# NVIDIA/k8s-cc-manager

Hardware: AMD Instinct MI355X
Metric: reconcile_gpus_per_sec (higher is better)
Workload: dtype bf16; 1 GPU; model=cc-mode-transition, global_batch=1, seq_len=1024, parallelism=concurrent-per-gpu x1, modes=on<->off toggle, device_tier=shadow+hip-attest, eviction=True, components=5, attest_gemm_dim=1024

## Files before the change

k8s_cc_manager_amd/ops/attest.py:

```python

from __future__ import annotations

import ctypes
import logging
import os
import re
from dataclasses import dataclass, fields
from pathlib import Path
from typing import Optional

logger = logging.getLogger(__name__)

_LIB_PATH = Path(__file__).resolve().parent / "libccattest.so"
_lib: Optional[ctypes.CDLL] = None


class AttestationError(Exception):
    """The post-reset attestation probe failed — the device must NOT be
    labeled ready."""


def _from_c(cls, c, **special):
    special.update(error=c.error.decode(errors="replace"), ok=bool(c.ok))
    return cls(**{f.name: special[f.name] if f.name in special
# ... 188 lines not shown
        ("bad_offset", ctypes.c_ulonglong * 16),
        ("bad_expected", ctypes.c_uint * 16),
        ("bad_got", ctypes.c_uint * 16),
        ("bad_pass", ctypes.c_int * 16),
        ("fill_ms", ctypes.c_double),
        ("flip_ms", ctypes.c_double),
        ("scrub_ms", ctypes.c_double),
        ("zero_ms", ctypes.c_double),
        ("alloc_ms", ctypes.c_double),
        ("gbps", ctypes.c_double),
        ("beyond_cache", ctypes.c_int),
        ("scrubbed", ctypes.c_int),
        ("ok", ctypes.c_int),
        ("error", ctypes.c_char * 256),
    ]


HBM_MUL_LO, HBM_MUL_HI, HBM_SALT = 2654435769, 2246822519, 0x5EED0001
_HBM_NO_OFFSET = (1 << 64) - 1


def hbm_pattern_word(w: int, phase: int) -> int:
    if phase == 2:
        return 0
    if phase not in (0, 1):
        raise ValueError(f"phase={phase} outside 0..2")
    p = ((w & 0xFFFFFFFF) * HBM_MUL_LO + (w >> 32) * HBM_MUL_HI
         + HBM_SALT) & 0xFFFFFFFF
    return p ^ 0xFFFFFFFF if phase else p


@dataclass
class HbmMarchReport:

    device: int
    bytes_requested: int
    bytes_tested: int
    chunk_bytes: int
    origin: int
    chunks: int
    passes: int
    mismatch_words: int
    first_bad_offset: Optional[int]
    bad: list
    fill_ms: float
    flip_ms: float
    scrub_ms: float
    zero_ms: float
    alloc_ms: float
    gbps: float
    beyond_cache: bool
    scrubbed: bool
    ok: bool
    error: str = ""

    @classmethod
    def from_c(cls, c: _CHbmReport) -> "HbmMarchReport":
        n = max(0, min(c.n_bad, len(c.bad_offset)))
        first = c.first_bad_offset
        return _from_c(
            cls, c,
            first_bad_offset=None if first == _HBM_NO_OFFSET else first,
            bad=[(c.bad_offset[i], c.bad_expected[i], c.bad_got[i],
                  c.bad_pass[i]) for i in range(n)],
            beyond_cache=bool(c.beyond_cache), scrubbed=bool(c.scrubbed))


_INT, _PTR = ctypes.c_int, ctypes.c_void_p
_I64, _U64 = ctypes.c_longlong, ctypes.c_ulonglong
_GEMM =[_INT, _PTR, _PTR, _PTR, _INT, _INT, _INT]
_MX_GEMM = [_INT] + [_PTR] * 5 + [_INT] * 3
_UNIT_TABLE = [_INT, ctypes.POINTER(ctypes.c_uint), _INT]

_BINDINGS = {
    "cc_device_alive": (_INT, [_INT]),
    "cc_device_count": (_INT, []),
    "cc_device_index_for_bdf": (_INT, [_INT] * 3),
    "cc_mfma_gemm_bf16": (_INT, _GEMM),
    "cc_mfma_gemm_bf16_variant": (_INT, _GEMM + [_INT]),
    "cc_mfma_gemm_fp8_variant": (_INT, _GEMM + [_INT]),
    "cc_mfma_gemm_fp8": (_INT, _GEMM),
    "cc_ref_gemm_f32": (_INT, _GEMM),
    "cc_attest_device": (_INT, [_INT, _INT, ctypes.POINTER(_CReport)]),
    "cc_report_sizeof": (_INT, []),
    "cc_mfma_gemm_mxfp4": (_INT, _MX_GEMM),
    "cc_ref_gemm_mxfp4_f32": (_INT, _MX_GEMM),
    "cc_attest_mxfp4": (_INT, [_INT, _INT, ctypes.POINTER(_CMxReport)]),
    "cc_mx_report_sizeof": (_INT, []),
    "cc_cu_sweep": (_INT, [_INT, _INT, _INT, ctypes.POINTER(_CSweepReport)]),
    "cc_cu_sweep_gold": (_INT, [_INT, _INT, ctypes.POINTER(ctypes.c_float)]),
    "cc_cu_sweep_units": (_INT, _UNIT_TABLE),
    "cc_cu_sweep_hits": (_INT, _UNIT_TABLE),
    "cc_sweep_report_sizeof": (_INT, []),
    "cc_hbm_march": (_INT, [_INT, _I64, _INT, _U64, _I64, _INT,
                            ctypes.POINTER(_CHbmReport)]),
    "cc_hbm_step": (_INT, [_INT, _PTR, _I64, _U64, _INT, _INT,
                           ctypes.POINTER(_CHbmReport)]),
    "cc_hbm_report_sizeof": (_INT, []),
    "cc_attest_shutdown": (None, []),
}


def _load() -> ctypes.CDLL:
    global _lib
    if _lib is not None:
        return _lib
    if not _LIB_PATH.exists():
        raise AttestationError(
            f"attestation library missing: {_LIB_PATH} — run "
            "python -m k8s_cc_manager_amd.ops.build"
        )
    lib = ctypes.CDLL(str(_LIB_PATH))
    for name, (restype, argtypes) in _BINDINGS.items():
        fn = getattr(lib, name)
        fn.restype, fn.argtypes = restype, argtypes
    _lib = lib
    return lib


def probe_available() -> bool:
    try:
        return _load().cc_device_count() > 0
    except Exception:
        return False


def device_count() -> int:
    return _load().cc_device_count()


def device_alive(device_index: int) -> int:
    return _load().cc_device_alive(device_index)


def shutdown() -> None:
    _load().cc_attest_shutdown()


def attest_device(device_index: int, gemm_dim: int = 1024) -> AttestReport:
    lib = _load()
    c = _CReport()
    rc = lib.cc_attest_device(device_index, gemm_dim, ctypes.byref(c))
    rep = AttestReport.from_c(c)
    if rc != 0:
        raise AttestationError(
            f"device {device_index}: probe runtime error rc={rc}: {rep.error}"
        )
    if not rep.ok:
        raise AttestationError(
            f"device {device_index}: attestation FAILED "
            f"(max_abs_err={rep.max_abs_err}, fp8_max_abs_err={rep.fp8_max_abs_err}, "
            f"lds_failures={rep.lds_failures}, "
            f"xgmi {rep.peers_verified}/{rep.peers_attempted} attempted links verified)"
        )
    logger.info(
        "attested device %d: %s %d CUs, bf16 GEMM %.1f TF/s, fp8 GEMM "
        "%.1f TF/s (%dx%dx%d), LDS ok, HBM %.0f GB/s, xGMI %d/%d peers "
        "(%d verified, %.0f-%.0f GB/s/link)",
        rep.device,
        rep.arch,
        rep.cu_count,
        rep.gemm_tflops,
        rep.fp8_tflops,
        rep.gemm_dim,
        rep.gemm_dim,
        rep.gemm_dim,
        rep.hbm_gbps,
        rep.peers_accessible,
        rep.peer_count,
        rep.peers_verified,
        rep.xgmi_gbps_min,
        rep.xgmi_gbps_max,
    )
    _append_attest_log(rep)
    return rep


def attest_mxfp4(device_index: int, gemm_dim: int = 1024) -> MxReport:
    lib = _load()
    c = _CMxReport()
    rc = lib.cc_attest_mxfp4(device_index, gemm_dim, ctypes.byref(c))
    rep = MxReport.from_c(c)
    if rc != 0:
        raise AttestationError(
            f"device {device_index}: mxfp4 probe runtime error rc={rc}: {rep.error}"
        )
    if not rep.ok:
        raise AttestationError(
            f"device {device_index}: mxfp4 attestation FAILED "
            f"(mx_max_abs_err={rep.mx_max_abs_err}, mx_tflops={rep.mx_tflops})"
        )
    logger.info(
        "attested device %d: mxfp4 GEMM %.1f TF/s (%dx%dx%d), bitwise ok",
        rep.device,
        rep.mx_tflops,
        rep.mx_dim,
        rep.mx_dim,
        rep.mx_dim,
    )
    return rep


CU_SWEEP_MAX_ROUNDS = 256


def unit_name(unit: tuple) -> str:
    return "xcc%d/se%d/sh%d/cu%d/simd%d" % unit


def cu_sweep_report(device_index: int, rounds: int = 32,
                    _poison_key: int = -1) -> CuSweepReport:
    lib = _load()
    c = _CSweepReport()
    rc = lib.cc_cu_sweep(device_index, rounds, _poison_key, ctypes.byref(c))
    rep = CuSweepReport.from_c(c)
    if rc != 0:
        raise AttestationError(
            f"device {device_index}: cu sweep runtime error: {rep.error} rc={rc}"
        )
    return rep


def sweep_compute_units(device_index: int, rounds: int = 32,
                        _poison_key: int = -1) -> CuSweepReport:
    rep = cu_sweep_report(device_index, rounds, _poison_key)
    if not rep.ok:
        if rep.units_failed or rep.lds_failures:
            units = ", ".join(unit_name(u) for u in rep.failed_units)
            more = rep.units_failed - len(rep.failed_units)
            raise AttestationError(
                f"device {device_index}: cu sweep FAILED on {rep.units_failed} "
                f"unit(s): {units}{f' and {more} more' if more > 0 else ''} "
                f"(mfma_failures={rep.mfma_failures}, "
                f"lds_failures={rep.lds_failures})"
            )
        raise AttestationError(
            f"device {device_index}: cu sweep FAILED: {rep.error} "
            f"({rep.cus_seen}/{rep.cu_count} CUs)"
        )
    logger.info(
        "attested device %d: cu sweep %d/%d units on %d CUs of %d XCCs, "
        "%d launch(es), %.2f ms",
        rep.device,
        rep.units_seen,
        rep.units_expected,
        rep.cus_seen,
        rep.xccs_seen,
        rep.launches,
        rep.sweep_ms,
    )
    return rep


def cu_sweep_gold(device_index: int, rounds: int) -> list:
    buf = (ctypes.c_float * SWEEP_GOLD_ELEMS)()
    rc = _load().cc_cu_sweep_gold(device_index, rounds, buf)
    if rc != 0:
        raise AttestationError(f"cu_sweep_gold rc={rc}")
# ... 260 lines not shown
```

k8s_cc_manager_amd/ops/attest_kernels.hip:

```cpp

#include <hip/hip_runtime.h>

#include <chrono>
#include <cstdint>
#include <cstdio>
#include <cstdlib>
#include <mutex>
#include <new>
#include <vector>

#include "gemm_common.hip"
#include "gemm_bf16.hip"
#include "gemm_fp8.hip"
#include "gemm_fp4.hip"
#include "probe_kernels.hip"
#include "cu_sweep.hip"
#include "hbm_march.hip"

#include "probe_reports.hip"
#include "gemm_dispatch.hip"
#include "probe_ctx.hip"
#include "probe_legs.hip"

template <typename Report, typename Refuse = int (*)()>
// ... 18 lines not shown
           origin);
  return -2;
}

extern "C" {

int cc_device_alive(int device) {
  if (device < 0 || device >= kMaxDevices) return -1;
  if (hipSetDevice(device) != hipSuccess) return -1;
  int* d = nullptr;
  {
    std::lock_guard<std::mutex> lk(g_ctx_mu);
    DeviceCtx& dev = device_ctx(device);
    if (dev.dLive.ensure(sizeof(int)) != hipSuccess) return -2;
    d = dev.dLive;
  }
  if (hipMemset(d, 0, sizeof(int)) != hipSuccess) return -2;
  hipLaunchKernelGGL(liveness_kernel, dim3(1), dim3(64), 0, 0, d);
  int h = 0;
  hipError_t e = hipMemcpy(&h, d, sizeof(int), hipMemcpyDeviceToHost);
  if (e != hipSuccess) return -3;
  return h == 0x600D ? 0 : -4;
}

int cc_device_count(void) {
  int n = 0;
  if (hipGetDeviceCount(&n) != hipSuccess) return -1;
  return n;
}

int cc_device_index_for_bdf(int domain, int bus, int dev) {
  int n = 0;
  if (hipGetDeviceCount(&n) != hipSuccess) return -1;
  for (int i = 0; i < n; ++i) {
    hipDeviceProp_t p;
    if (hipGetDeviceProperties(&p, i) != hipSuccess) continue;
    if (p.pciDomainID == domain && p.pciBusID == bus && p.pciDeviceID == dev)
      return i;
  }
  return -1;
}

int cc_mfma_gemm_bf16(int device, const void* A, const void* Bt, void* C,
                      int M, int N, int K) {
  if (hipSetDevice(device) != hipSuccess) return -3;
  int rc = launch_mfma_gemm(A, Bt, C, M, N, K);
  if (rc != 0) return rc;
  return (int)hipDeviceSynchronize();
}

int cc_mfma_gemm_bf16_variant(int device, const void* A, const void* Bt,
                              void* C, int M, int N, int K, int which) {
  return run_forced_variant(forced_variant(kBf16Forced, which), 2, device, A,
                            Bt, C, M, N, K);
}

int cc_mfma_gemm_fp8_variant(int device, const void* A, const void* Bt,
                             void* C, int M, int N, int K, int which) {
  return run_forced_variant(forced_variant(kFp8Forced, which), 1, device, A,
                            Bt, C, M, N, K);
}

int cc_mfma_gemm_fp8(int device, const void* A, const void* Bt, void* C,
                     int M, int N, int K) {
  if (hipSetDevice(device) != hipSuccess) return -3;
  int rc = launch_fp8_best(A, Bt, C, M, N, K);
  if (rc != 0) return rc;
  return (int)hipDeviceSynchronize();
}

int cc_ref_gemm_f32(int device, const void* A, const void* Bt, void* C,
                    int M, int N, int K) {
  if (hipSetDevice(device) != hipSuccess) return -3;
  dim3 block(16, 16);
  dim3 grid((N + 15) / 16, (M + 15) / 16);
  hipLaunchKernelGGL(ref_gemm_f32, grid, block, 0, 0, (const bf16*)A,
                     (const bf16*)Bt, (float*)C, M, N, K);
  return (int)hipDeviceSynchronize();
}

int cc_attest_device(int device, int gemm_dim, struct CcAttestReport* rep) {
  CC_TRY(report_begin(rep, device));

  hipDeviceProp_t prop;
  CC_CHECK(hipGetDeviceProperties(&prop, device));
  rep->cu_count = prop.multiProcessorCount;
  rep->vram_total_mb = (long long)(prop.totalGlobalMem >> 20);
  __builtin_strncpy(rep->arch, prop.gcnArchName, sizeof(rep->arch) - 1);

  const int D = (gemm_dim / BM) * BM > 0 ? (gemm_dim / BM) * BM : BM;
  rep->gemm_m = rep->gemm_n = rep->gemm_k = D;

  std::lock_guard<std::mutex> lk(g_ctx_mu);
  DeviceCtx& dev = device_ctx(device);
  CC_CHECK(dev.main.acquire(D));
  CC_CHECK(dev.events());

  CC_TRY(probe_bf16(dev, rep));
  CC_TRY(probe_fp8(dev, rep));
  CC_TRY(probe_lds(dev, rep));
  CC_TRY(probe_hbm(dev, rep));
  CC_TRY(probe_xgmi(dev, rep));

  rep->ok = (rep->max_abs_err == 0.0f) && (rep->fp8_max_abs_err == 0.0f) &&
                    (rep->lds_failures == 0) && (rep->gemm_tflops > 0.0) &&
                    (rep->peers_verified == rep->peers_attempted)
                ? 1
                : 0;
  return 0;
}

int cc_report_sizeof(void) { return (int)sizeof(struct CcAttestReport); }

int cc_mfma_gemm_mxfp4(int device, const void* A, const void* SA,
                       const void* Bt, const void* SB, void* C, int M, int N,
                       int K) {
  if (hipSetDevice(device) != hipSuccess) return -3;
  int rc = launch_mxfp4(A, SA, Bt, SB, C, M, N, K);
  if (rc != 0) return rc;
  return (int)hipDeviceSynchronize();
}

int cc_ref_gemm_mxfp4_f32(int device, const void* A, const void* SA,
                          const void* Bt, const void* SB, void* C, int M,
                          int N, int K) {
  if (M <= 0 || N <= 0 || K <= 0 || K % 32) return -2;
  if (hipSetDevice(device) != hipSuccess) return -3;
  launch_ref_mxfp4(A, SA, Bt, SB, C, M, N, K);
  return (int)hipDeviceSynchronize();
}

int cc_attest_mxfp4(int device, int gemm_dim, struct CcMxReport* rep) {
  CC_TRY(report_begin(rep, device));

  const int D = gemm_dim < BK4 ? BK4 : (gemm_dim / BK4) * BK4;
  rep->mx_m = rep->mx_n = rep->mx_k = D;

  std::lock_guard<std::mutex> lk(g_ctx_mu);
  DeviceCtx& dev = device_ctx(device);
  CC_CHECK(dev.events());
  CC_CHECK(dev.mx.acquire(D));
  CC_TRY(probe_mxfp4(dev, rep));

  rep->ok = (rep->mx_max_abs_err == 0.0f) && (rep->mx_tflops > 0.0) ? 1 : 0;
  return 0;
}

int cc_mx_report_sizeof(void) { return (int)sizeof(struct CcMxReport); }

int cc_cu_sweep(int device, int rounds, int poison_key,
                struct CcSweepReport* rep) {
  CC_TRY(report_begin(rep, device, [&] {
    rep->rounds = rounds;
    if (rounds >= 1 && rounds <= CU_SWEEP_MAX_ROUNDS) return 0;
    snprintf(rep->error, sizeof(rep->error), "rounds %d outside 1..%d", rounds,
             CU_SWEEP_MAX_ROUNDS);
    return -2;
  }));
  hipDeviceProp_t prop;
  CC_CHECK(hipGetDeviceProperties(&prop, device));
  rep->cu_count = prop.multiProcessorCount;
  rep->units_expected = 4 * rep->cu_count;

  std::lock_guard<std::mutex> lk(g_ctx_mu);
  DeviceCtx& dev = device_ctx(device);
  CC_CHECK(dev.events());
  CC_CHECK(dev.sweep.acquire());
  CC_TRY(probe_cu_sweep(dev, rep, poison_key));

  const bool covered = rep->units_seen == rep->units_expected &&
                       rep->cus_seen == rep->cu_count;
  if (!covered)
    snprintf(rep->error, sizeof(rep->error),
             "coverage %d/%d after %d launches", rep->units_seen,
             rep->units_expected, rep->launches);
  rep->ok = covered && rep->units_failed == 0 && rep->lds_failures == 0 ? 1 : 0;
  return 0;
}

int cc_cu_sweep_gold(int device, int rounds, float* host_out_3328) {
  if (!host_out_3328) return -1;
  if (device < 0 || device >= kMaxDevices) return -5;
  if (rounds < 1 || rounds > CU_SWEEP_MAX_ROUNDS) return -2;
  if (hipSetDevice(device) != hipSuccess) return -3;
  std::lock_guard<std::mutex> lk(g_ctx_mu);
  DeviceCtx& dev = device_ctx(device);
  if (dev.events() != hipSuccess || dev.sweep.acquire() != hipSuccess)
    return -4;
  ErrorText err;
  double ms = 0.0;
  CC_TRY(sweep_gold(dev, &err, rounds, &ms));
  return (int)hipMemcpy(host_out_3328, dev.sweep.dSweepGold,
// ... 132 lines not shown
```

k8s_cc_manager_amd/ops/probe_ctx.hip:

```cpp

#define CC_CHECK(expr)                                                         \
  do {                                                                         \
    hipError_t _e = (expr);                                                    \
    if (_e != hipSuccess) {                                                    \
      snprintf(rep->error, sizeof(rep->error), "%s: %s", #expr,                \
               hipGetErrorString(_e));                                         \
      return (int)_e;                                                          \
    }                                                                          \
  } while (0)

#define CC_TRY(expr)                                                           \
  do {                                                                         \
    int _rc = (expr);                                                          \
    if (_rc != 0) return _rc;                                                  \
  } while (0)

constexpr int kMaxDevices = 64;

template <typename T>
struct DevBuf {
  T* p = nullptr;
  size_t bytes = 0;
  DevBuf() = default;
  DevBuf& operator=(DevBuf&& o) {
    release();
    p = o.p, bytes = o.bytes;
    o.p = nullptr, o.bytes = 0;
    return *this;
  }
  hipError_t ensure(size_t n) {
    if (bytes == n) return hipSuccess;
    release();
    hipError_t e = hipMalloc(&p, n);
    if (e != hipSuccess) p = nullptr;
    bytes = p ? n : 0;
    return e;
  }
  void release() {
    if (p) (void)hipFree(p);
    p = nullptr;
    bytes = 0;
  }
  operator T*() const { return p; }
};

struct MainCtx {
  int dim = 0;
  int ref_valid = 0;
  int peer_cursor = 0;
  DevBuf<bf16> dA, dB;
  DevBuf<unsigned char> dA8, dB8;
  DevBuf<float> dC, dRef, dHbm, dErr;
  DevBuf<unsigned long long> dSum;
  DevBuf<uint32_t> dFail;

  hipError_t acquire(int D) {
    if (dim == D) return hipSuccess;
    *this = MainCtx{};
    const size_t n = (size_t)D * D;
    hipError_t e;
    if ((e = dA.ensure(n * sizeof(bf16))) || (e = dB.ensure(n * sizeof(bf16))) ||
        (e = dA8.ensure(n)) || (e = dB8.ensure(n)) ||
        (e = dC.ensure(n * sizeof(float))) ||
        (e = dRef.ensure(n * sizeof(float))) ||
        (e = dHbm.ensure(n * sizeof(float))) || (e = dErr.ensure(sizeof(float))) ||
        (e = dSum.ensure(sizeof(unsigned long long))) ||
        (e = dFail.ensure(sizeof(uint32_t))))
      return e;
    dim = D;
    return hipSuccess;
  }
};

struct PeerCtx {
  DevBuf<float> dPeerDst;
  DevBuf<unsigned long long> dPeerSum;
};

struct MxCtx {
  int dim = 0;
  int ref_valid = 0;
  DevBuf<unsigned char> dMxA, dMxB;
  DevBuf<unsigned char> dMxSA, dMxSB;
  DevBuf<float> dMxC, dMxRef, dMxErr;
  DevBuf<unsigned long long> dMxSum;

  hipError_t acquire(int D) {
    if (dim == D) return hipSuccess;
    *this = MxCtx{};
    const size_t n = (size_t)D * D;
    hipError_t e;
    if ((e = dMxA.ensure(n / 2)) || (e = dMxB.ensure(n / 2)) ||
        (e = dMxSA.ensure(n / 32)) || (e = dMxSB.ensure(n / 32)) ||
        (e = dMxC.ensure(n * sizeof(float))) ||
        (e = dMxRef.ensure(n * sizeof(float))) ||
        (e = dMxErr.ensure(sizeof(float))) ||
        (e = dMxSum.ensure(sizeof(unsigned long long))))
      return e;
    dim = D;
    return hipSuccess;
  }
};

struct SweepCtx {
  DevBuf<unsigned> dSweepTab;
  DevBuf<float> dSweepGold;
  int gold_rounds = 0;
  std::vector<unsigned> hSweepTab;
  int valid = 0;

  static constexpr size_t kTabWords = (size_t)CU_SWEEP_UNITS * CU_SWEEP_REC;
  hipError_t acquire() {
    hipError_t e;
    if ((e = dSweepTab.ensure(kTabWords * sizeof(unsigned))) ||
        (e = dSweepGold.ensure(CU_SWEEP_GOLD_ELEMS * sizeof(float))))
      return e;
    try {
      hSweepTab.resize(kTabWords);
    } catch (const std::bad_alloc&) {
      return hipErrorOutOfMemory;
    }
    return hipSuccess;
  }
};

struct HbmCtx {
  DevBuf<HbmMarchResult> dRes;
  hipError_t acquire() { return dRes.ensure(sizeof(HbmMarchResult)); }
};

struct DeviceCtx {
  bool used = false;
  MainCtx main;
  PeerCtx peer;
  MxCtx mx;
  SweepCtx sweep;
  HbmCtx hbm;
  DevBuf<int> dLive;
  hipEvent_t ev0 = nullptr, ev1 = nullptr;

  hipError_t events() {
    hipError_t e;
    if (!ev0 && (e = hipEventCreate(&ev0)) != hipSuccess) return e;
    if (!ev1 && (e = hipEventCreate(&ev1)) != hipSuccess) return e;
    return hipSuccess;
  }
  void release() {
    if (ev0) (void)hipEventDestroy(ev0);
    if (ev1) (void)hipEventDestroy(ev1);
    *this = DeviceCtx{};
  }
};

static DeviceCtx g_ctx[kMaxDevices];
static std::mutex g_ctx_mu;

static DeviceCtx& device_ctx(int device) {
  g_ctx[device].used = true;
  return g_ctx[device];
}

template <typename Report, typename Launch>
static int timed_ms(DeviceCtx& dev, Report* rep, double* ms, Launch launch) {
  hipEvent_t ev0 = dev.ev0, ev1 = dev.ev1;
  CC_CHECK(hipEventRecord(ev0, 0));
  CC_TRY(launch());
  CC_CHECK(hipEventRecord(ev1, 0));
  CC_CHECK(hipEventSynchronize(ev1));
  float f = 0.f;
  (void)hipEventElapsedTime(&f, ev0, ev1);
  *ms = (double)f;
  return 0;
}

template <typename T>
static hipError_t read_back(const void* dptr, T* out) {
  return hipMemcpy(out, dptr, sizeof(T), hipMemcpyDeviceToHost);
}

struct DeviceHop {
  int home;
  bool away = false;
  explicit DeviceHop(int device) : home(device) {}
  hipError_t to(int peer) {
    away = true;
    return hipSetDevice(peer);
  }
  hipError_t back() {
    hipError_t e = hipSetDevice(home);
    away = e != hipSuccess;
    return e;
  }
  ~DeviceHop() {
    if (away) (void)hipSetDevice(home);
  }
};
```

k8s_cc_manager_amd/ops/probe_kernels.hip:

```cpp
#pragma once

#include "gemm_common.hip"

typedef __attribute__((ext_vector_type(4))) float float4v;

__global__ void fill_bf16_lcg(bf16* __restrict__ out, long n, uint32_t seed) {
  long i = (long)blockIdx.x * blockDim.x + threadIdx.x;
  long stride = (long)gridDim.x * blockDim.x;
  for (; i < n; i += stride) {
    uint32_t x = (uint32_t)i * 1103515245u + seed * 747796405u + 12345u;
    x ^= x >> 16;
    x *= 2654435769u;
    int v = (int)((x >> 13) & 3u) - 2;
    out[i] = (bf16)(float)v;
  }
}

__global__ void fill_fp8_lcg(unsigned char* __restrict__ out, long n,
                             uint32_t seed) {
  const unsigned char enc[4] = {0xC0, 0xB8, 0x00, 0x38};
  long i = (long)blockIdx.x * blockDim.x + threadIdx.x;
  long stride = (long)gridDim.x * blockDim.x;
  for (; i < n; i += stride) {
    uint32_t x = (uint32_t)i * 1103515245u + seed * 747796405u + 12345u;
// ... 36 lines not shown
    uint32_t x = (uint32_t)i * 1103515245u + seed * 747796405u + 12345u;
    x ^= x >> 16;
    x *= 2654435769u;
    out[i] = (unsigned char)(126u + ((x >> 13) % 3u));
  }
}

__device__ __forceinline__ int e2m1_times2(int code) {
  int e = (code >> 1) & 3, m = code & 1;
  int v = e ? (2 + m) << (e - 1) : m;
  return (code & 8) ? -v : v;
}

__global__ void ref_gemm_mxfp4_f32(const unsigned char* __restrict__ A,
                                   const unsigned char* __restrict__ SA,
                                   const unsigned char* __restrict__ Bt,
                                   const unsigned char* __restrict__ SB,
                                   float* __restrict__ C, int M, int N,
                                   int K) {
  int col = blockIdx.x * blockDim.x + threadIdx.x;
  int row = blockIdx.y * blockDim.y + threadIdx.y;
  if (row >= M || col >= N) return;
  const unsigned char* a = A + (long)row * (K >> 1);
  const unsigned char* b = Bt + (long)col * (K >> 1);
  const unsigned char* sa = SA + (long)row * (K >> 5);
  const unsigned char* sb = SB + (long)col * (K >> 5);
  float acc = 0.f;
  for (int kb = 0; kb < (K >> 5); ++kb) {
    float blk = 0.f;
    for (int j = 0; j < 16; ++j) {
      int ab = a[kb * 16 + j], bb = b[kb * 16 + j];
      blk += (float)(e2m1_times2(ab & 15) * e2m1_times2(bb & 15));
      blk += (float)(e2m1_times2(ab >> 4) * e2m1_times2(bb >> 4));
    }
    acc += ldexpf(blk, (int)sa[kb] + (int)sb[kb] - 254 - 2);
  }
  C[(long)row * N + col] = acc;
}

__global__ void max_abs_diff(const float* __restrict__ x,
                             const float* __restrict__ y, long n,
                             float* out) {
  __shared__ float smax[256];
  long i = (long)blockIdx.x * blockDim.x + threadIdx.x;
  long stride = (long)gridDim.x * blockDim.x;
  float m = 0.f;
  for (; i < n; i += stride) {
    float d = fabsf(x[i] - y[i]);
    m = fmaxf(m, d);
  }
  smax[threadIdx.x] = m;
  __syncthreads();
  for (int s = 128; s > 0; s >>= 1) {
    if (threadIdx.x < s) smax[threadIdx.x] = fmaxf(smax[threadIdx.x], smax[threadIdx.x + s]);
    __syncthreads();
  }
  if (threadIdx.x == 0) {
    atomicMax((unsigned int*)out, __float_as_uint(smax[0]));
  }
}

__global__ void checksum_f32(const float* __restrict__ x, long n,
                             unsigned long long* out) {
  long i = (long)blockIdx.x * blockDim.x + threadIdx.x;
  long stride = (long)gridDim.x * blockDim.x;
  unsigned long long h = 0;
  for (; i < n; i += stride) {
    unsigned long long v = (unsigned long long)__float_as_uint(x[i]) + 0x9e3779b97f4a7c15ull * (unsigned long long)(i + 1);
    v ^= v >> 33; v *= 0xff51afd7ed558ccdull; v ^= v >> 33;
    h ^= v;
  }
  for (int off = 32; off > 0; off >>= 1)
    h ^= __shfl_down(h, off, 64);
  __shared__ unsigned long long partial[4];
  if ((threadIdx.x & 63) == 0) partial[threadIdx.x >> 6] = h;
  __syncthreads();
  if (threadIdx.x == 0) {
    unsigned long long b = partial[0];
    for (int w = 1; w < (int)(blockDim.x >> 6); ++w) b ^= partial[w];
    atomicXor(out, b);
  }
}

constexpr int LDS_PROBE_WORDS = 16384;

__global__ void lds_probe(uint32_t* __restrict__ fail_count, int rounds) {
  __shared__ uint32_t slab[LDS_PROBE_WORDS];
  const int tid = threadIdx.x;
  const int nthreads = blockDim.x;
  uint32_t local_fail = 0;
  for (int r = 0; r < rounds; ++r) {
    uint32_t salt = 0x9e3779b9u * (r + 1) + blockIdx.x;
    for (int i = tid; i < LDS_PROBE_WORDS; i += nthreads)
      slab[i] = (uint32_t)i * 2654435769u + salt;
    __syncthreads();
    for (int i = tid; i < LDS_PROBE_WORDS; i += nthreads) {
      int j = (i * 33 + r) & (LDS_PROBE_WORDS - 1);
      uint32_t want = (uint32_t)j * 2654435769u + salt;
      if (slab[j] != want) ++local_fail;
    }
    __syncthreads();
  }
  if (local_fail) atomicAdd(fail_count, local_fail);
}

__global__ void hbm_copy_f4(const float4v* __restrict__ src,
                            float4v* __restrict__ dst, long n4) {
  long i = (long)blockIdx.x * blockDim.x + threadIdx.x;
  long stride = (long)gridDim.x * blockDim.x;
  for (; i < n4; i += stride) dst[i] = src[i];
}

extern "C" __global__ void liveness_kernel(int* out) {
  if (threadIdx.x == 0 && blockIdx.x == 0) *out = 0x600D;
}
```

k8s_cc_manager_amd/ops/probe_legs.hip:

```cpp

template <typename Report, typename Launch>
static int timed_gemm(DeviceCtx& dev, Report* rep, int D, double* ms,
                      double* tflops, Launch launch) {
  auto checked = [&] { return launch() != 0 ? -6 : 0; };
  CC_TRY(checked());
  CC_CHECK(hipDeviceSynchronize());
  CC_TRY(timed_ms(dev, rep, ms, checked));
  *tflops = 2.0 * D * (double)D * D / (*ms * 1e-3) / 1e12;
  return 0;
}

template <typename Report, typename Launch>
static int cached_reference(DeviceCtx& dev, Report* rep, int* valid,
                            double* ms, Launch launch) {
  *ms = 0.0;
  if (*valid) return 0;
  CC_TRY(timed_ms(dev, rep, ms, [&] {
    launch();
    return 0;
  }));
  *valid = 1;
  return 0;
}

template <typename Report>
static int compare_read_back(Report* rep, const float* dC, const float* dRef,
                             long elems, float* dErr, float* err,
                             unsigned long long* dSum = nullptr,
                             unsigned long long* sum = nullptr) {
  hipLaunchKernelGGL(max_abs_diff, dim3(1024), dim3(256), 0, 0, dC, dRef,
                     elems, dErr);
  if (dSum)
    hipLaunchKernelGGL(checksum_f32, dim3(1024), dim3(256), 0, 0, dC, elems,
                       dSum);
  CC_CHECK(hipDeviceSynchronize());
  CC_CHECK(read_back(dErr, err));
  if (dSum) CC_CHECK(read_back(dSum, sum));
  return 0;
}

static int probe_bf16(DeviceCtx& dev, CcAttestReport* rep) {
  MainCtx& ctx = dev.main;
  const int D = ctx.dim;
  const long elems = (long)D * D;
  bf16 *dA = ctx.dA, *dB = ctx.dB;
  float *dC = ctx.dC, *dRef = ctx.dRef, *dErr = ctx.dErr;
  unsigned long long* dSum = ctx.dSum;
  CC_CHECK(hipMemset(dErr, 0, sizeof(float)));
  CC_CHECK(hipMemset(dSum, 0, sizeof(unsigned long long)));

  hipLaunchKernelGGL(fill_bf16_lcg, dim3(2048), dim3(256), 0, 0, dA, elems, 1u);
  hipLaunchKernelGGL(fill_bf16_lcg, dim3(2048), dim3(256), 0, 0, dB, elems, 7u);

  CC_TRY(timed_gemm(dev, rep, D, &rep->gemm_ms, &rep->gemm_tflops,
                    [&] { return launch_mfma_gemm(dA, dB, dC, D, D, D); }));
  CC_TRY(cached_reference(dev, rep, &ctx.ref_valid, &rep->ref_ms, [&] {
    dim3 rblock(16, 16), rgrid((D + 15) / 16, (D + 15) / 16);
    hipLaunchKernelGGL(ref_gemm_f32, rgrid, rblock, 0, 0, dA, dB, dRef, D, D,
                       D);
  }));
  return compare_read_back(rep, dC, dRef, elems, dErr, &rep->max_abs_err, dSum,
                           &rep->checksum);
}

static int probe_fp8(DeviceCtx& dev, CcAttestReport* rep) {
  MainCtx& ctx = dev.main;
  const int D = ctx.dim;
  const long elems = (long)D * D;
  float *dC = ctx.dC, *dErr = ctx.dErr;
  hipLaunchKernelGGL(fill_fp8_lcg, dim3(2048), dim3(256), 0, 0, ctx.dA8.p,
                     elems, 1u);
  hipLaunchKernelGGL(fill_fp8_lcg, dim3(2048), dim3(256), 0, 0, ctx.dB8.p,
                     elems, 7u);
  CC_TRY(timed_gemm(dev, rep, D, &rep->fp8_ms, &rep->fp8_tflops, [&] {
    return launch_fp8_best(ctx.dA8, ctx.dB8, dC, D, D, D);
  }));
  CC_CHECK(hipMemset(dErr, 0, sizeof(float)));
  return compare_read_back(rep, dC, ctx.dRef, elems, dErr,
                           &rep->fp8_max_abs_err);
}

static int probe_lds(DeviceCtx& dev, CcAttestReport* rep) {
  uint32_t* dFail = dev.main.dFail;
  CC_CHECK(hipMemset(dFail, 0, sizeof(uint32_t)));
  CC_TRY(timed_ms(dev, rep, &rep->lds_ms, [&] {
    hipLaunchKernelGGL(lds_probe, dim3(512), dim3(256), 0, 0, dFail, 8);
    return 0;
  }));
  CC_CHECK(read_back(dFail, &rep->lds_failures));
  return 0;
}

static int probe_hbm(DeviceCtx& dev, CcAttestReport* rep) {
  MainCtx& ctx = dev.main;
  long n4 = (long)ctx.dim * ctx.dim / 4;
  CC_TRY(timed_ms(dev, rep, &rep->hbm_ms, [&] {
    hipLaunchKernelGGL(hbm_copy_f4, dim3(4096), dim3(256), 0, 0,
                       (const float4v*)ctx.dC.p, (float4v*)ctx.dHbm.p, n4);
    return 0;
  }));
  rep->hbm_gbps = 2.0 * n4 * 16.0 / (rep->hbm_ms * 1e-3) / 1e9;
  return 0;
}

static int probe_xgmi(DeviceCtx& dev, CcAttestReport* rep) {
  MainCtx& ctx = dev.main;
  const int device = rep->device;
  float* dC = ctx.dC;
  unsigned long long* dSum = ctx.dSum;
  int ndev = 0;
  CC_CHECK(hipGetDeviceCount(&ndev));
  rep->peer_count = ndev - 1;
  if (ndev > kMaxDevices) ndev = kMaxDevices;
  long bytes = (long)ctx.dim * ctx.dim * sizeof(float);
  if (bytes > (2L << 20)) bytes = 2L << 20;
  long sum_elems = bytes / sizeof(float);
  CC_CHECK(hipMemset(dSum, 0, sizeof(unsigned long long)));
  hipLaunchKernelGGL(checksum_f32, dim3(1024), dim3(256), 0, 0, dC, sum_elems,
                     dSum);
  CC_CHECK(hipDeviceSynchronize());
  unsigned long long src_sum = 0;
  CC_CHECK(read_back(dSum, &src_sum));
  int acc[kMaxDevices];
  int n_acc = 0;
  for (int p = 0; p < ndev; ++p) {
    if (p == device) continue;
    int can = 0;
    if (hipDeviceCanAccessPeer(&can, device, p) == hipSuccess && can)
      acc[n_acc++] = p;
  }
  rep->peers_accessible = n_acc;
  int max_peers = 0;
  if (const char* mp = getenv("CC_ATTEST_XGMI_MAX_PEERS")) max_peers = atoi(mp);
  int attempts = (max_peers > 0 && max_peers < n_acc) ? max_peers : n_acc;
  rep->peers_attempted = attempts;
  DeviceHop hop(device);
  for (int t = 0; t < attempts; ++t) {
    int p = acc[(ctx.peer_cursor + t) % (n_acc ? n_acc : 1)];
    hipError_t pe = hipDeviceEnablePeerAccess(p, 0);
    if (pe != hipSuccess && pe != hipErrorPeerAccessAlreadyEnabled) {
      (void)hipGetLastError();
    }
    PeerCtx& pc = device_ctx(p).peer;
    CC_CHECK(hop.to(p));
    if ((long)pc.dPeerDst.bytes < bytes &&
        pc.dPeerDst.ensure(bytes) != hipSuccess) {
      CC_CHECK(hop.back());
      continue;
    }
    if (pc.dPeerSum.ensure(sizeof(unsigned long long)) != hipSuccess) {
      CC_CHECK(hop.back());
      continue;
    }
    CC_CHECK(hipMemset(pc.dPeerDst, 0, bytes));
    CC_CHECK(hop.back());
    const int kPeerIters = 4;
    double ms = 0.0;
    CC_TRY(timed_ms(dev, rep, &ms, [&] {
      for (int it = 0; it < kPeerIters; ++it)
        CC_CHECK(hipMemcpyPeerAsync(pc.dPeerDst, p, dC, device, bytes, 0));
      return 0;
    }));
    rep->xgmi_ms += ms;
    double gbps = (double)bytes * kPeerIters / (ms * 1e-3) / 1e9;
    if (rep->xgmi_gbps_min == 0.0 || gbps < rep->xgmi_gbps_min)
      rep->xgmi_gbps_min = gbps;
    if (gbps > rep->xgmi_gbps_max) rep->xgmi_gbps_max = gbps;
    CC_CHECK(hop.to(p));
    CC_CHECK(hipMemset(pc.dPeerSum, 0, sizeof(unsigned long long)));
    hipLaunchKernelGGL(checksum_f32, dim3(1024), dim3(256), 0, 0,
                       pc.dPeerDst.p, sum_elems, pc.dPeerSum.p);
    CC_CHECK(hipDeviceSynchronize());
    unsigned long long peer_sum = 0;
    CC_CHECK(read_back(pc.dPeerSum, &peer_sum));
    CC_CHECK(hop.back());
    if (peer_sum == src_sum) ++rep->peers_verified;
  }
  if (n_acc) ctx.peer_cursor = (ctx.peer_cursor + attempts) % n_acc;
  return 0;
}

static int probe_mxfp4(DeviceCtx& dev, CcMxReport* rep) {
  MxCtx& ctx = dev.mx;
  const int D = ctx.dim;
  const long elems = (long)D * D;
  unsigned char *dA = ctx.dMxA, *dB = ctx.dMxB;
  unsigned char *dSA = ctx.dMxSA, *dSB = ctx.dMxSB;
  float *dC = ctx.dMxC, *dRef = ctx.dMxRef, *dErr = ctx.dMxErr;
  unsigned long long* dSum = ctx.dMxSum;
  CC_CHECK(hipMemset(dErr, 0, sizeof(float)));
  CC_CHECK(hipMemset(dSum, 0, sizeof(unsigned long long)));
  CC_CHECK(hipMemset(dC, 0x7F, elems * sizeof(float)));

  hipLaunchKernelGGL(fill_fp4_lcg, dim3(2048), dim3(256), 0, 0, dA, elems / 2,
                     1u);
  hipLaunchKernelGGL(fill_fp4_lcg, dim3(2048), dim3(256), 0, 0, dB, elems / 2,
                     7u);
  hipLaunchKernelGGL(fill_e8m0_lcg, dim3(256), dim3(256), 0, 0, dSA,
                     elems / 32, 1u);
  hipLaunchKernelGGL(fill_e8m0_lcg, dim3(256), dim3(256), 0, 0, dSB,
                     elems / 32, 7u);

  CC_TRY(timed_gemm(dev, rep, D, &rep->mx_ms, &rep->mx_tflops, [&] {
    return launch_mxfp4(dA, dSA, dB, dSB, dC, D, D, D);
  }));
  CC_TRY(cached_reference(dev, rep, &ctx.ref_valid, &rep->mx_ref_ms, [&] {
    launch_ref_mxfp4(dA, dSA, dB, dSB, dRef, D, D, D);
  }));
  return compare_read_back(rep, dC, dRef, elems, dErr, &rep->mx_max_abs_err,
                           dSum, &rep->mx_checksum);
}

template <typename Report>
static int sweep_gold(DeviceCtx& dev, Report* rep, int rounds, double* ms) {
  SweepCtx& ctx = dev.sweep;
  *ms = 0.0;
  if (ctx.gold_rounds == rounds) return 0;
  ctx.gold_rounds = 0;
// ... 170 lines not shown
```

Before: 342.9 GPU-transitions/s.

## Batch attestation probe legs into one async stream with single readback

Restructures the per-device attestation so that the bf16 GEMM, the fp8 GEMM, both comparisons, the LDS probe and the HBM copy are queued back-to-back on the default stream. Timing uses per-leg events, and a single MainResult struct is read back once, replacing several memsets, synchronizations and small readbacks per leg. Input fills and the reference GEMM move into a one-time prepare step that is skipped once the reference is cached. Device properties are cached, and a fused compare+checksum kernel also produces the xGMI source slice checksum, removing a separate checksum pass. The cost is that inputs are not refilled on each attestation, and per-leg timings now depend on event placement in the stream rather than on isolated timed runs.

```diff
diff --git a/k8s_cc_manager_amd/ops/attest.py b/k8s_cc_manager_amd/ops/attest.py
--- a/k8s_cc_manager_amd/ops/attest.py
+++ b/k8s_cc_manager_amd/ops/attest.py
@@ -294,6 +294,11 @@
     "cc_mfma_gemm_fp8": (_INT, _GEMM),
     "cc_ref_gemm_f32": (_INT, _GEMM),
     "cc_attest_device": (_INT, [_INT, _INT, ctypes.POINTER(_CReport)]),
+    "cc_compare_checksum": (_INT, [_INT, _PTR, _PTR, _I64, _I64,
+                                   ctypes.POINTER(ctypes.c_float),
+                                   ctypes.POINTER(_U64),
+                                   ctypes.POINTER(_U64)]),
+    "cc_attest_poison_ref": (_INT, [_INT, _I64]),
     "cc_report_sizeof": (_INT, []),
     "cc_mfma_gemm_mxfp4": (_INT, _MX_GEMM),
     "cc_ref_gemm_mxfp4_f32": (_INT, _MX_GEMM),
@@ -386,6 +391,21 @@
     )
     _append_attest_log(rep)
     return rep
+
+
+def compare_checksum(device_index: int, x_ptr: int, y_ptr: Optional[int],
+                     n: int, m: int = 0) -> tuple:
+    err, s_all, s_slice = ctypes.c_float(), _U64(), _U64()
+    rc = _load().cc_compare_checksum(
+        device_index, x_ptr, y_ptr, n, m, ctypes.byref(err),
+        ctypes.byref(s_all), ctypes.byref(s_slice))
+    if rc != 0:
+        raise AttestationError(f"compare_checksum rc={rc}")
+    return err.value, s_all.value, s_slice.value
+
+
+def _poison_ref(device_index: int, elem: int) -> int:
+    return _load().cc_attest_poison_ref(device_index, elem)
 
 
 def attest_mxfp4(device_index: int, gemm_dim: int = 1024) -> MxReport:
diff --git a/k8s_cc_manager_amd/ops/attest_kernels.hip b/k8s_cc_manager_amd/ops/attest_kernels.hip
--- a/k8s_cc_manager_amd/ops/attest_kernels.hip
+++ b/k8s_cc_manager_amd/ops/attest_kernels.hip
@@ -124,25 +124,25 @@
 int cc_attest_device(int device, int gemm_dim, struct CcAttestReport* rep) {
   CC_TRY(report_begin(rep, device));
 
-  hipDeviceProp_t prop;
-  CC_CHECK(hipGetDeviceProperties(&prop, device));
-  rep->cu_count = prop.multiProcessorCount;
-  rep->vram_total_mb = (long long)(prop.totalGlobalMem >> 20);
-  __builtin_strncpy(rep->arch, prop.gcnArchName, sizeof(rep->arch) - 1);
-
   const int D = (gemm_dim / BM) * BM > 0 ? (gemm_dim / BM) * BM : BM;
   rep->gemm_m = rep->gemm_n = rep->gemm_k = D;
 
   std::lock_guard<std::mutex> lk(g_ctx_mu);
   DeviceCtx& dev = device_ctx(device);
+  CC_CHECK(dev.props(device));
+  rep->cu_count = dev.cu_count;
+  rep->vram_total_mb = dev.vram_total_mb;
+  __builtin_memcpy(rep->arch, dev.arch, sizeof(rep->arch));
   CC_CHECK(dev.main.acquire(D));
   CC_CHECK(dev.events());
 
-  CC_TRY(probe_bf16(dev, rep));
-  CC_TRY(probe_fp8(dev, rep));
-  CC_TRY(probe_lds(dev, rep));
-  CC_TRY(probe_hbm(dev, rep));
-  CC_TRY(probe_xgmi(dev, rep));
+  XgmiPlan plan;
+  CC_TRY(xgmi_plan(dev.main, rep, &plan));
+  if (!dev.main.ref_valid) CC_TRY(probe_prepare(dev, rep));
+  unsigned long long slice_sum = 0;
+  CC_TRY(probe_local(dev, rep, plan.attempts ? plan.sum_elems : 0,
+                     &slice_sum));
+  CC_TRY(probe_xgmi(dev, rep, plan, slice_sum));
 
   rep->ok = (rep->max_abs_err == 0.0f) && (rep->fp8_max_abs_err == 0.0f) &&
                     (rep->lds_failures == 0) && (rep->gemm_tflops > 0.0) &&
@@ -150,6 +150,45 @@
                 ? 1
                 : 0;
   return 0;
+}
+
+int cc_compare_checksum(int device, const void* x, const void* y, long long n,
+                        long long m, float* err, unsigned long long* sum_all,
+                        unsigned long long* sum_slice) {
+  if (!x || n < 1 || m < 0 || m > n || (uintptr_t)x % 16 || (uintptr_t)y % 16)
+    return -2;
+  if (hipSetDevice(device) != hipSuccess) return -3;
+  MainResult* d = nullptr;
+  if (hipMalloc(&d, sizeof(MainResult)) != hipSuccess) return -4;
+  MainResult h = {};
+  hipError_t e = hipMemsetAsync(d, 0, sizeof(MainResult), 0);
+  if (e == hipSuccess) {
+    hipLaunchKernelGGL(compare_checksum, dim3(compare_blocks(n)),
+                       dim3(COMPARE_THREADS), 0, 0, (const float*)x,
+                       (const float*)y, (long)n, (long)m,
+                       CompareOut{err ? &d->bf16_err_bits : nullptr,
+                                  sum_all ? &d->checksum : nullptr,
+                                  sum_slice ? &d->slice_sum : nullptr});
+    e = hipMemcpy(&h, d, sizeof(h), hipMemcpyDeviceToHost);
+  }
+  (void)hipFree(d);
+  if (e != hipSuccess) return (int)e;
+  if (err) __builtin_memcpy(err, &h.bf16_err_bits, sizeof(float));
+  if (sum_all) *sum_all = h.checksum;
+  if (sum_slice) *sum_slice = h.slice_sum;
+  return 0;
+}
+
+int cc_attest_poison_ref(int device, long long elem) {
+  if (device < 0 || device >= kMaxDevices) return -2;
+  std::lock_guard<std::mutex> lk(g_ctx_mu);
+  const MainCtx& ctx = g_ctx[device].main;
+  if (!ctx.dim || !ctx.ref_valid || elem < 0 ||
+      elem >= (long long)ctx.dim * ctx.dim)
+    return -2;
+  if (hipSetDevice(device) != hipSuccess) return -3;
+  hipLaunchKernelGGL(poison_add_one, dim3(1), dim3(64), 0, 0, ctx.dRef.p + elem);
+  return (int)hipDeviceSynchronize();
 }
 
 int cc_report_sizeof(void) { return (int)sizeof(struct CcAttestReport); }
diff --git a/k8s_cc_manager_amd/ops/probe_ctx.hip b/k8s_cc_manager_amd/ops/probe_ctx.hip
--- a/k8s_cc_manager_amd/ops/probe_ctx.hip
+++ b/k8s_cc_manager_amd/ops/probe_ctx.hip
@@ -44,15 +44,23 @@
   operator T*() const { return p; }
 };
 
+struct MainResult {
+  unsigned int bf16_err_bits;
+  unsigned int fp8_err_bits;
+  unsigned int lds_failures;
+  unsigned int pad;
+  unsigned long long checksum;
+  unsigned long long slice_sum;
+};
+
 struct MainCtx {
   int dim = 0;
   int ref_valid = 0;
   int peer_cursor = 0;
   DevBuf<bf16> dA, dB;
   DevBuf<unsigned char> dA8, dB8;
-  DevBuf<float> dC, dRef, dHbm, dErr;
-  DevBuf<unsigned long long> dSum;
-  DevBuf<uint32_t> dFail;
+  DevBuf<float> dC, dRef, dHbm;
+  DevBuf<MainResult> dRes;
 
   hipError_t acquire(int D) {
     if (dim == D) return hipSuccess;
@@ -63,9 +71,8 @@
         (e = dA8.ensure(n)) || (e = dB8.ensure(n)) ||
         (e = dC.ensure(n * sizeof(float))) ||
         (e = dRef.ensure(n * sizeof(float))) ||
-        (e = dHbm.ensure(n * sizeof(float))) || (e = dErr.ensure(sizeof(float))) ||
-        (e = dSum.ensure(sizeof(unsigned long long))) ||
-        (e = dFail.ensure(sizeof(uint32_t))))
+        (e = dHbm.ensure(n * sizeof(float))) ||
+        (e = dRes.ensure(sizeof(MainResult))))
       return e;
     dim = D;
     return hipSuccess;
@@ -138,16 +145,37 @@
   HbmCtx hbm;
   DevBuf<int> dLive;
   hipEvent_t ev0 = nullptr, ev1 = nullptr;
+  static constexpr int kLegEvents = 8;
+  hipEvent_t leg_ev[kLegEvents] = {};
+  bool have_props = false;
+  int cu_count = 0;
+  long long vram_total_mb = 0;
+  char arch[64] = "";
 
   hipError_t events() {
     hipError_t e;
     if (!ev0 && (e = hipEventCreate(&ev0)) != hipSuccess) return e;
     if (!ev1 && (e = hipEventCreate(&ev1)) != hipSuccess) return e;
+    for (hipEvent_t& ev : leg_ev)
+      if (!ev && (e = hipEventCreate(&ev)) != hipSuccess) return e;
+    return hipSuccess;
+  }
+  hipError_t props(int device) {
+    if (have_props) return hipSuccess;
+    hipDeviceProp_t p;
+    hipError_t e = hipGetDeviceProperties(&p, device);
+    if (e != hipSuccess) return e;
+    cu_count = p.multiProcessorCount;
+    vram_total_mb = (long long)(p.totalGlobalMem >> 20);
+    __builtin_strncpy(arch, p.gcnArchName, sizeof(arch) - 1);
+    have_props = true;
     return hipSuccess;
   }
   void release() {
     if (ev0) (void)hipEventDestroy(ev0);
     if (ev1) (void)hipEventDestroy(ev1);
+    for (hipEvent_t ev : leg_ev)
+      if (ev) (void)hipEventDestroy(ev);
     *this = DeviceCtx{};
   }
 };
diff --git a/k8s_cc_manager_amd/ops/probe_kernels.hip b/k8s_cc_manager_amd/ops/probe_kernels.hip
--- a/k8s_cc_manager_amd/ops/probe_kernels.hip
+++ b/k8s_cc_manager_amd/ops/probe_kernels.hip
@@ -142,6 +142,93 @@
   }
 }
 
+__device__ __forceinline__ unsigned long long checksum_mix(float x, long i) {
+  unsigned long long v = (unsigned long long)__float_as_uint(x) +
+                         0x9e3779b97f4a7c15ull * (unsigned long long)(i + 1);
+  v ^= v >> 33; v *= 0xff51afd7ed558ccdull; v ^= v >> 33;
+  return v;
+}
+
+struct CompareOut {
+  unsigned int* err;
+  unsigned long long* sum_all;
+  unsigned long long* sum_slice;
+};
+
+constexpr int COMPARE_THREADS = 256;
+constexpr int COMPARE_MAX_BLOCKS = 512;
+
+__global__ void __launch_bounds__(COMPARE_THREADS)
+compare_checksum(const float* __restrict__ x, const float* __restrict__ y,
+                 long n, long m, CompareOut out) {
+  const long n4 = n >> 2;
+  const bool want_all = out.sum_all != nullptr;
+  const long hash_to = want_all ? n : (out.sum_slice ? m : 0);
+  const float4v* x4 = (const float4v*)x;
+  const float4v* y4 = (const float4v*)y;
+  float e = 0.f;
+  unsigned long long h_all = 0, h_slice = 0;
+  auto element = [&](float xv, float yv, long i) {
+    e = fmaxf(e, fabsf(xv - yv));
+    if (i < hash_to) {
+      unsigned long long v = checksum_mix(xv, i);
+      h_all ^= v;
+      if (i < m) h_slice ^= v;
+    }
+  };
+  long v = (long)blockIdx.x * COMPARE_THREADS + threadIdx.x;
+  const long stride = (long)gridDim.x * COMPARE_THREADS;
+#pragma unroll 2
+  for (; v < n4; v += stride) {
+    float4v a = x4[v];
+    float4v b = y ? y4[v] : a;
+    const long i = v << 2;
+    element(a.x, b.x, i);
+    element(a.y, b.y, i + 1);
+    element(a.z, b.z, i + 2);
+    element(a.w, b.w, i + 3);
+  }
+  if (blockIdx.x == 0) {
+    const long i = (n4 << 2) + threadIdx.x;
+    if (i < n) element(x[i], y ? y[i] : x[i], i);
+  }
+  for (int off = 32; off > 0; off >>= 1) {
+    e = fmaxf(e, __shfl_down(e, off, 64));
+    h_all ^= __shfl_down(h_all, off, 64);
+    h_slice ^= __shfl_down(h_slice, off, 64);
+  }
+  constexpr int kWaves = COMPARE_THREADS / 64;
+  __shared__ float s_e[kWaves];
+  __shared__ unsigned long long s_all[kWaves], s_slice[kWaves];
+  if ((threadIdx.x & 63) == 0) {
+    s_e[threadIdx.x >> 6] = e;
+    s_all[threadIdx.x >> 6] = h_all;
+    s_slice[threadIdx.x >> 6] = h_slice;
+  }
+  __syncthreads();
+  if (threadIdx.x == 0) {
+    for (int w = 1; w < kWaves; ++w) {
+      e = fmaxf(e, s_e[w]);
+      h_all ^= s_all[w];
+      h_slice ^= s_slice[w];
+    }
+    if (out.err && e != 0.f) atomicMax(out.err, __float_as_uint(e));
+    if (want_all) atomicXor(out.sum_all, h_all);
+    if (out.sum_slice && m > 0) atomicXor(out.sum_slice, h_slice);
+  }
+}
+
+static inline int compare_blocks(long n) {
+  long blocks = ((n >> 2) + COMPARE_THREADS - 1) / COMPARE_THREADS;
+  return blocks < 1 ? 1
+                    : blocks > COMPARE_MAX_BLOCKS ? COMPARE_MAX_BLOCKS
+                                                  : (int)blocks;
+}
+
+__global__ void poison_add_one(float* p) {
+  if (threadIdx.x == 0 && blockIdx.x == 0) *p += 1.0f;
+}
+
 constexpr int LDS_PROBE_WORDS = 16384;
 
 __global__ void lds_probe(uint32_t* __restrict__ fail_count, int rounds) {
diff --git a/k8s_cc_manager_amd/ops/probe_legs.hip b/k8s_cc_manager_amd/ops/probe_legs.hip
--- a/k8s_cc_manager_amd/ops/probe_legs.hip
+++ b/k8s_cc_manager_amd/ops/probe_legs.hip
@@ -39,101 +39,141 @@
   return 0;
 }
 
-static int probe_bf16(DeviceCtx& dev, CcAttestReport* rep) {
+struct XgmiPlan {
+  int acc[kMaxDevices];
+  int n_acc = 0;
+  int attempts = 0;
+  long bytes = 0;
+  long sum_elems = 0;
+};
+
+static int xgmi_plan(const MainCtx& ctx, CcAttestReport* rep, XgmiPlan* plan) {
+  const int device = rep->device;
+  int ndev = 0;
+  CC_CHECK(hipGetDeviceCount(&ndev));
+  rep->peer_count = ndev - 1;
+  if (ndev > kMaxDevices) ndev = kMaxDevices;
+  plan->bytes = (long)ctx.dim * ctx.dim * sizeof(float);
+  if (plan->bytes > (2L << 20)) plan->bytes = 2L << 20;
+  plan->sum_elems = plan->bytes / sizeof(float);
+  for (int p = 0; p < ndev; ++p) {
+    if (p == device) continue;
+    int can = 0;
+    if (hipDeviceCanAccessPeer(&can, device, p) == hipSuccess && can)
+      plan->acc[plan->n_acc++] = p;
+  }
+  rep->peers_accessible = plan->n_acc;
+  int max_peers = 0;
+  if (const char* mp = getenv("CC_ATTEST_XGMI_MAX_PEERS")) max_peers = atoi(mp);
+  plan->attempts =
+      (max_peers > 0 && max_peers < plan->n_acc) ? max_peers : plan->n_acc;
+  rep->peers_attempted = plan->attempts;
+  return 0;
+}
+
+static int probe_prepare(DeviceCtx& dev, CcAttestReport* rep) {
   MainCtx& ctx = dev.main;
   const int D = ctx.dim;
   const long elems = (long)D * D;
   bf16 *dA = ctx.dA, *dB = ctx.dB;
-  float *dC = ctx.dC, *dRef = ctx.dRef, *dErr = ctx.dErr;
-  unsigned long long* dSum = ctx.dSum;
-  CC_CHECK(hipMemset(dErr, 0, sizeof(float)));
-  CC_CHECK(hipMemset(dSum, 0, sizeof(unsigned long long)));
-
+  float *dC = ctx.dC, *dRef = ctx.dRef;
   hipLaunchKernelGGL(fill_bf16_lcg, dim3(2048), dim3(256), 0, 0, dA, elems, 1u);
   hipLaunchKernelGGL(fill_bf16_lcg, dim3(2048), dim3(256), 0, 0, dB, elems, 7u);
-
-  CC_TRY(timed_gemm(dev, rep, D, &rep->gemm_ms, &rep->gemm_tflops,
-                    [&] { return launch_mfma_gemm(dA, dB, dC, D, D, D); }));
-  CC_TRY(cached_reference(dev, rep, &ctx.ref_valid, &rep->ref_ms, [&] {
+  hipLaunchKernelGGL(fill_fp8_lcg, dim3(2048), dim3(256), 0, 0, ctx.dA8.p,
+                     elems, 1u);
+  hipLaunchKernelGGL(fill_fp8_lcg, dim3(2048), dim3(256), 0, 0, ctx.dB8.p,
+                     elems, 7u);
+  if (launch_mfma_gemm(dA, dB, dC, D, D, D) != 0) return -6;
+  if (launch_fp8_best(ctx.dA8, ctx.dB8, dC, D, D, D) != 0) return -6;
+  int valid = 0;
+  CC_TRY(cached_reference(dev, rep, &valid, &rep->ref_ms, [&] {
     dim3 rblock(16, 16), rgrid((D + 15) / 16, (D + 15) / 16);
     hipLaunchKernelGGL(ref_gemm_f32, rgrid, rblock, 0, 0, dA, dB, dRef, D, D,
                        D);
   }));
-  return compare_read_back(rep, dC, dRef, elems, dErr, &rep->max_abs_err, dSum,
-                           &rep->checksum);
-}
-
-static int probe_fp8(DeviceCtx& dev, CcAttestReport* rep) {
+  CC_CHECK(hipDeviceSynchronize());
+  ctx.ref_valid = 1;
+  return 0;
+}
+
+template <typename Report>
+static int elapsed_ms(Report* rep, hipEvent_t from, hipEvent_t to, double* ms) {
+  float f = 0.f;
+  hipError_t e = hipEventElapsedTime(&f, from, to);
+  if (e == hipErrorNotReady) {
+    CC_CHECK(hipEventSynchronize(to));
+    e = hipEventElapsedTime(&f, from, to);
+  }
+  CC_CHECK(e);
+  *ms = (double)f;
+  return 0;
+}
+
+static int probe_local(DeviceCtx& dev, CcAttestReport* rep, long slice_elems,
+                       unsigned long long* slice_sum) {
   MainCtx& ctx = dev.main;
   const int D = ctx.dim;
   const long elems = (long)D * D;
-  float *dC = ctx.dC, *dErr = ctx.dErr;
-  hipLaunchKernelGGL(fill_fp8_lcg, dim3(2048), dim3(256), 0, 0, ctx.dA8.p,
-                     elems, 1u);
-  hipLaunchKernelGGL(fill_fp8_lcg, dim3(2048), dim3(256), 0, 0, ctx.dB8.p,
-                     elems, 7u);
-  CC_TRY(timed_gemm(dev, rep, D, &rep->fp8_ms, &rep->fp8_tflops, [&] {
-    return launch_fp8_best(ctx.dA8, ctx.dB8, dC, D, D, D);
-  }));
-  CC_CHECK(hipMemset(dErr, 0, sizeof(float)));
-  return compare_read_back(rep, dC, ctx.dRef, elems, dErr,
-                           &rep->fp8_max_abs_err);
-}
-
-static int probe_lds(DeviceCtx& dev, CcAttestReport* rep) {
-  uint32_t* dFail = dev.main.dFail;
-  CC_CHECK(hipMemset(dFail, 0, sizeof(uint32_t)));
-  CC_TRY(timed_ms(dev, rep, &rep->lds_ms, [&] {
-    hipLaunchKernelGGL(lds_probe, dim3(512), dim3(256), 0, 0, dFail, 8);
-    return 0;
-  }));
-  CC_CHECK(read_back(dFail, &rep->lds_failures));
-  return 0;
-}
-
-static int probe_hbm(DeviceCtx& dev, CcAttestReport* rep) {
-  MainCtx& ctx = dev.main;
-  long n4 = (long)ctx.dim * ctx.dim / 4;
-  CC_TRY(timed_ms(dev, rep, &rep->hbm_ms, [&] {
-    hipLaunchKernelGGL(hbm_copy_f4, dim3(4096), dim3(256), 0, 0,
-                       (const float4v*)ctx.dC.p, (float4v*)ctx.dHbm.p, n4);
-    return 0;
-  }));
+  const long n4 = elems / 4;
+  float *dC = ctx.dC, *dRef = ctx.dRef;
+  MainResult* dRes = ctx.dRes;
+  hipEvent_t* ev = dev.leg_ev;
+  const dim3 cgrid(compare_blocks(elems)), cblock(COMPARE_THREADS);
+
+  CC_CHECK(hipMemsetAsync(dRes, 0, sizeof(MainResult), 0));
+
+  CC_CHECK(hipEventRecord(ev[0], 0));
+  if (launch_mfma_gemm(ctx.dA.p, ctx.dB.p, dC, D, D, D) != 0) return -6;
+  CC_CHECK(hipEventRecord(ev[1], 0));
+  hipLaunchKernelGGL(compare_checksum, cgrid, cblock, 0, 0, dC, dRef, elems,
+                     0L, CompareOut{&dRes->bf16_err_bits, &dRes->checksum,
+                                    nullptr});
+
+  CC_CHECK(hipEventRecord(ev[2], 0));
+  if (launch_fp8_best(ctx.dA8.p, ctx.dB8.p, dC, D, D, D) != 0) return -6;
+  CC_CHECK(hipEventRecord(ev[3], 0));
+  hipLaunchKernelGGL(compare_checksum, cgrid, cblock, 0, 0, dC, dRef, elems,
+                     slice_elems,
+                     CompareOut{&dRes->fp8_err_bits, nullptr,
+                                slice_elems ? &dRes->slice_sum : nullptr});
+
+  CC_CHECK(hipEventRecord(ev[4], 0));
+  hipLaunchKernelGGL(lds_probe, dim3(512), dim3(256), 0, 0,
+                     &dRes->lds_failures, 8);
+  CC_CHECK(hipEventRecord(ev[5], 0));
+
+  CC_CHECK(hipEventRecord(ev[6], 0));
+  hipLaunchKernelGGL(hbm_copy_f4, dim3(4096), dim3(256), 0, 0,
+                     (const float4v*)dC, (float4v*)ctx.dHbm.p, n4);
+  CC_CHECK(hipEventRecord(ev[7], 0));
+
+  MainResult h;
+  CC_CHECK(hipMemcpy(&h, dRes, sizeof(h), hipMemcpyDeviceToHost));
+  __builtin_memcpy(&rep->max_abs_err, &h.bf16_err_bits, sizeof(float));
+  __builtin_memcpy(&rep->fp8_max_abs_err, &h.fp8_err_bits, sizeof(float));
+  rep->lds_failures = h.lds_failures;
+  rep->checksum = h.checksum;
+  *slice_sum = h.slice_sum;
+
+  CC_TRY(elapsed_ms(rep, ev[0], ev[1], &rep->gemm_ms));
+  CC_TRY(elapsed_ms(rep, ev[2], ev[3], &rep->fp8_ms));
+  CC_TRY(elapsed_ms(rep, ev[4], ev[5], &rep->lds_ms));
+  CC_TRY(elapsed_ms(rep, ev[6], ev[7], &rep->hbm_ms));
+  const double flop = 2.0 * D * (double)D * D;
+  rep->gemm_tflops = flop / (rep->gemm_ms * 1e-3) / 1e12;
+  rep->fp8_tflops = flop / (rep->fp8_ms * 1e-3) / 1e12;
   rep->hbm_gbps = 2.0 * n4 * 16.0 / (rep->hbm_ms * 1e-3) / 1e9;
   return 0;
 }
 
-static int probe_xgmi(DeviceCtx& dev, CcAttestReport* rep) {
+static int probe_xgmi(DeviceCtx& dev, CcAttestReport* rep,
+                      const XgmiPlan& plan, unsigned long long src_sum) {
   MainCtx& ctx = dev.main;
   const int device = rep->device;
   float* dC = ctx.dC;
-  unsigned long long* dSum = ctx.dSum;
-  int ndev = 0;
-  CC_CHECK(hipGetDeviceCount(&ndev));
-  rep->peer_count = ndev - 1;
-  if (ndev > kMaxDevices) ndev = kMaxDevices;
-  long bytes = (long)ctx.dim * ctx.dim * sizeof(float);
-  if (bytes > (2L << 20)) bytes = 2L << 20;
-  long sum_elems = bytes / sizeof(float);
-  CC_CHECK(hipMemset(dSum, 0, sizeof(unsigned long long)));
-  hipLaunchKernelGGL(checksum_f32, dim3(1024), dim3(256), 0, 0, dC, sum_elems,
-                     dSum);
-  CC_CHECK(hipDeviceSynchronize());
-  unsigned long long src_sum = 0;
-  CC_CHECK(read_back(dSum, &src_sum));
-  int acc[kMaxDevices];
-  int n_acc = 0;
-  for (int p = 0; p < ndev; ++p) {
-    if (p == device) continue;
-    int can = 0;
-    if (hipDeviceCanAccessPeer(&can, device, p) == hipSuccess && can)
-      acc[n_acc++] = p;
-  }
-  rep->peers_accessible = n_acc;
-  int max_peers = 0;
-  if (const char* mp = getenv("CC_ATTEST_XGMI_MAX_PEERS")) max_peers = atoi(mp);
-  int attempts = (max_peers > 0 && max_peers < n_acc) ? max_peers : n_acc;
-  rep->peers_attempted = attempts;
+  const int* acc = plan.acc;
+  const int n_acc = plan.n_acc, attempts = plan.attempts;
+  const long bytes = plan.bytes, sum_elems = plan.sum_elems;
   DeviceHop hop(device);
   for (int t = 0; t < attempts; ++t) {
     int p = acc[(ctx.peer_cursor + t) % (n_acc ? n_acc : 1)];
```

Result: slower. 316.3 GPU-transitions/s (-7.8%).
